# lbcb-sci/raven

Hardware: NVIDIA H100
Metric: overlaps/s (higher is better)
Workload: dtype u64

## Files before the change

raven_b200/csrc/map.cu:

```cuda
#include <algorithm>

#include "engine.cuh"

namespace rvn {

namespace {

constexpr int kThreads = 256;

struct IndexView {
  ValView val;
  const uint64_t* org;
  const uint32_t* bucket;
  uint64_t n;
  int shift;
  uint32_t occurrence;
  uint64_t limit;
};

__device__ __forceinline__ void Lookup(const IndexView& ix, uint64_t v,
                                       uint32_t* first, uint32_t* count) {
  if (v > ix.limit) {
    *first = 0;
    *count = 0;
// ... 39 lines not shown

__global__ void __launch_bounds__(kThreads)
ProbeKernel(IndexView ix, ValView q_val,
            const uint64_t* __restrict__ q_org, uint64_t q_begin, uint64_t n_q,
            bool avoid_equal, bool avoid_symmetric,
            uint32_t* __restrict__ cnt, uint32_t* __restrict__ first,
            uint8_t* __restrict__ filt) {
  const uint64_t i = static_cast<uint64_t>(blockIdx.x) * kThreads + threadIdx.x;
  if (i >= n_q) return;
  const uint64_t v = q_val[q_begin + i];
  const uint32_t lhs_id = static_cast<uint32_t>(q_org[q_begin + i] >> 32);
  uint32_t f, n;
  Lookup(ix, v, &f, &n);
  uint32_t kept = 0;
  uint8_t over = 0;
  if (n > ix.occurrence) {
    over = 1;
    n = 0;
  } else {
    for (uint32_t j = 0; j < n; ++j) {
      kept += KeepPosting(lhs_id, ix.org[f + j], avoid_equal, avoid_symmetric);
    }
  }
  cnt[i] = kept;
  first[i] = f;
  filt[i] = over;
}

__global__ void __launch_bounds__(kThreads)
ExpandKernel(IndexView ix, ValView q_val,
             const uint64_t* __restrict__ q_org, uint64_t q_begin, uint64_t n_q,
             bool avoid_equal, bool avoid_symmetric,
             const uint32_t* __restrict__ cnt,
             const uint32_t* __restrict__ first,
             const uint64_t* __restrict__ hit_off, uint64_t* __restrict__ h_grp,
             uint64_t* __restrict__ h_pos) {
  const uint64_t i = static_cast<uint64_t>(blockIdx.x) * kThreads + threadIdx.x;
  if (i >= n_q) return;
  uint32_t left = cnt[i];
  if (left == 0) return;
  const uint64_t v = q_val[q_begin + i];
  const uint64_t lo = q_org[q_begin + i];
  const uint32_t lhs_id = static_cast<uint32_t>(lo >> 32);
  const uint64_t lhs_pos = static_cast<uint32_t>(lo) >> 1;
  uint64_t dst = hit_off[i];
  for (uint64_t j = first[i]; left > 0 && j < ix.n && ix.val[j] == v; ++j) {
    const uint64_t o = ix.org[j];
    if (!KeepPosting(lhs_id, o, avoid_equal, avoid_symmetric)) continue;
    const uint64_t rhs_id = o >> 32;
    const uint64_t strand = (lo & 1) == (o & 1);
    const uint64_t rhs_pos = static_cast<uint32_t>(o) >> 1;
    const uint64_t diagonal =
        !strand ? rhs_pos + lhs_pos : rhs_pos - lhs_pos + (3ULL << 30);
    h_grp[dst] = (((rhs_id << 1) | strand) << 32) | diagonal;
    h_pos[dst] = (lhs_pos << 32) | rhs_pos;
    ++dst;
    --left;
  }
}

__global__ void __launch_bounds__(kThreads)
ProbeSuffixKernel(IndexView ix, ValView q_val,
                  const uint64_t* __restrict__ q_org, uint64_t q_begin, uint64_t n_q,
                  bool strict_above, uint32_t* __restrict__ cnt,
                  uint32_t* __restrict__ first, uint8_t* __restrict__ filt) {
  const uint64_t i = static_cast<uint64_t>(blockIdx.x) * kThreads + threadIdx.x;
  if (i >= n_q) return;
  const uint64_t v = q_val[q_begin + i];
  uint32_t f, n;
  Lookup(ix, v, &f, &n);
  uint8_t over = 0;
  uint32_t kept = 0, fk = f;
  if (n > ix.occurrence) {
    over = 1;
  } else if (n > 0) {
    if (strict_above) {
      const uint32_t lhs_id = static_cast<uint32_t>(q_org[q_begin + i] >> 32);
      uint32_t lo = f, hi = f + n;
      while (lo < hi) {
        const uint32_t mid = lo + (hi - lo) / 2;
        if (static_cast<uint32_t>(ix.org[mid] >> 32) <= lhs_id) lo = mid + 1; else hi = mid;
      }
      fk = lo;
    }
    kept = f + n - fk;
  }
  cnt[i] = kept;
  first[i] = fk;
  filt[i] = over;
}

__global__ void __launch_bounds__(kThreads)
ProbeSortedKernel(IndexView ix, ValView sorted_val,
                  const uint32_t* __restrict__ sorted_idx,
                  const uint64_t* __restrict__ q_org, uint64_t q_begin, uint64_t n_q,
                  bool strict_above, uint64_t* __restrict__ packed) {
  const uint64_t t = static_cast<uint64_t>(blockIdx.x) * kThreads + threadIdx.x;
  if (t >= n_q) return;
  const uint64_t v = sorted_val[t];
  const uint32_t i = sorted_idx[t];
  uint32_t f, n;
  Lookup(ix, v, &f, &n);
  uint8_t over = 0;
  uint32_t kept = 0, fk = f;
  if (n > ix.occurrence) {
    over = 1;
  } else if (n > 0) {
    if (strict_above) {
      const uint32_t lhs_id = static_cast<uint32_t>(q_org[q_begin + i] >> 32);
      uint32_t lo = f, hi = f + n;
      while (lo < hi) {
        const uint32_t mid = lo + (hi - lo) / 2;
        if (static_cast<uint32_t>(ix.org[mid] >> 32) <= lhs_id) lo = mid + 1; else hi = mid;
      }
      fk = lo;
    }
    kept = f + n - fk;
  }
  packed[i] = (static_cast<uint64_t>(fk) << 32) | (static_cast<uint64_t>(over) << 31) | kept;
}

__global__ void UnpackProbe(const uint64_t* __restrict__ packed, uint64_t n,
                            uint32_t* __restrict__ cnt, uint32_t* __restrict__ first,
                            uint8_t* __restrict__ filt) {
  const uint64_t i = static_cast<uint64_t>(blockIdx.x) * blockDim.x + threadIdx.x;
  if (i >= n) return;
  const uint64_t p = packed[i];
  cnt[i] = static_cast<uint32_t>(p) & 0x7FFFFFFFu;
  first[i] = static_cast<uint32_t>(p >> 32);
  filt[i] = static_cast<uint8_t>((p >> 31) & 1);
}


__global__ void __launch_bounds__(kThreads)
ExpandWarpKernel(IndexView ix, const uint64_t* __restrict__ q_org, uint64_t q_begin,
                 uint64_t n_q, const uint32_t* __restrict__ cnt,
                 const uint32_t* __restrict__ first, const uint64_t* __restrict__ hit_off,
                 uint64_t* __restrict__ h_grp, uint64_t* __restrict__ h_pos) {
  const uint32_t lane = threadIdx.x & 31;
  const uint64_t i = (static_cast<uint64_t>(blockIdx.x) * kThreads + threadIdx.x);
  const bool valid = i < n_q;
  const uint32_t my_cnt = valid ? cnt[i] : 0;
  const uint32_t my_first = valid ? first[i] : 0;
  const uint64_t my_org = valid ? q_org[q_begin + i] : 0;
  const uint64_t my_off = valid ? hit_off[i] : 0;
  const uint64_t base = __shfl_sync(0xFFFFFFFFu, my_off, 0);
  uint32_t rel = valid ? static_cast<uint32_t>(my_off - base) : 0;
  uint32_t run = valid ? rel + my_cnt : 0;
  for (int d = 1; d < 32; d <<= 1) {
    const uint32_t o = __shfl_up_sync(0xFFFFFFFFu, run, d);
    if (lane >= d && o > run) run = o;
  }
  if (!valid) rel = run;
  const uint32_t total = __shfl_sync(0xFFFFFFFFu, run, 31);
  for (uint32_t t0 = 0; t0 < total; t0 += 32) {
    const uint32_t t = t0 + lane;
    uint32_t q = 0;
#pragma unroll
    for (uint32_t step = 16; step > 0; step >>= 1) {
      const uint32_t r = __shfl_sync(0xFFFFFFFFu, rel, q + step);
      if (r <= t) q += step;
    }
    const uint32_t qrel = __shfl_sync(0xFFFFFFFFu, rel, q);
    const uint32_t qfirst = __shfl_sync(0xFFFFFFFFu, my_first, q);
    const uint64_t lo = __shfl_sync(0xFFFFFFFFu, my_org, q);
    if (t < total) {
      const uint64_t o = ix.org[qfirst + (t - qrel)];
      const uint64_t lhs_pos = static_cast<uint32_t>(lo) >> 1;
      const uint64_t rhs_id = o >> 32;
      const uint64_t strand = (lo & 1) == (o & 1);
      const uint64_t rhs_pos = static_cast<uint32_t>(o) >> 1;
      const uint64_t diagonal =
          !strand ? rhs_pos + lhs_pos : rhs_pos - lhs_pos + (3ULL << 30);
      h_grp[base + t] = (((rhs_id << 1) | strand) << 32) | diagonal;
      h_pos[base + t] = (lhs_pos << 32) | rhs_pos;
    }
  }
}

struct JoinView {
  ValView val;
  const uint64_t* org;
  uint64_t n;
  uint32_t occurrence;
  const uint64_t* thr_val;
  const uint32_t* thr_pos;
  uint32_t first, last;
};

__device__ __forceinline__ bool JoinIsQuery(const JoinView& jv, uint64_t v, uint64_t o) {
  const uint32_t r = static_cast<uint32_t>(o >> 32);
  if (r < jv.first || r >= jv.last) return false;
  const uint64_t t = jv.thr_val[r - jv.first];
  return v < t || (v == t && (static_cast<uint32_t>(o) >> 1) < jv.thr_pos[r - jv.first]);
}

template <typename Pred>
__device__ __forceinline__ uint64_t WarpFirst(uint64_t lo, uint64_t hi, uint32_t lane,
                                              Pred past) {
  while (lo < hi) {
    const uint64_t step = (hi - lo + 31) / 32;
    const uint64_t p = lo + (lane + 1) * step - 1;
    const uint32_t b = __ballot_sync(0xFFFFFFFFu, p >= hi || past(p));
    if (!b) return hi;
    const uint64_t f = __ffs(b) - 1;
    hi = min(hi, lo + (f + 1) * step - 1);
    lo += f * step;
  }
  return lo;
}

__global__ void __launch_bounds__(kThreads)
JoinSweepKernel(JoinView jv, const uint64_t* __restrict__ q_off,
                uint32_t* __restrict__ cursor, uint64_t* __restrict__ packed) {
  constexpr uint32_t kAll = 0xFFFFFFFFu;
  const uint32_t lane = threadIdx.x & 31;
  const uint64_t base = (static_cast<uint64_t>(blockIdx.x) * kThreads + threadIdx.x) & ~31ULL;
  if (base >= jv.n) return;
  const uint64_t i = base + lane;
  const bool valid = i < jv.n;
  const uint64_t v = valid ? jv.val[i] : 0;
  const uint64_t o = valid ? jv.org[i] : 0;
  const uint32_t r = static_cast<uint32_t>(o >> 32);
  const bool q = valid && JoinIsQuery(jv, v, o);
  if (!__any_sync(kAll, q)) return;

  uint64_t vn = __shfl_down_sync(kAll, v, 1);
  uint32_t rn = __shfl_down_sync(kAll, r, 1);
  uint64_t vp = __shfl_up_sync(kAll, v, 1);
  const bool has_next = i + 1 < jv.n;
  if (lane == 31 && has_next) {
    vn = jv.val[i + 1];
    rn = static_cast<uint32_t>(jv.org[i + 1] >> 32);
  }
  if (lane == 0 && i > 0) vp = jv.val[i - 1];
  const bool run_tail = !has_next || vn != v;
  const uint32_t tails = __ballot_sync(kAll, run_tail);
  const uint32_t seg_tails = __ballot_sync(kAll, run_tail || rn != r);
  const uint32_t heads = __ballot_sync(kAll, i == 0 || vp != v);
  const uint32_t at_or_above = kAll << lane, at_or_below = kAll >> (31 - lane);
  uint64_t run_end = (tails & at_or_above) ? base + __ffs(tails & at_or_above) : 0;
  uint64_t seg_end = (seg_tails & at_or_above) ? base + __ffs(seg_tails & at_or_above) : 0;
  bool over = false;
  const bool limited = jv.occurrence != kAll;

  if (__any_sync(kAll, q && run_end == 0)) {
    const uint64_t vl = __shfl_sync(kAll, v, 31);
    const uint32_t rl = __shfl_sync(kAll, r, 31);
    const uint64_t j = base + 32, k = j + lane;
    const bool dv = k >= jv.n || jv.val[k] != vl;
    const uint32_t bv = __ballot_sync(kAll, dv);
    const uint32_t bs =
        __ballot_sync(kAll, dv || static_cast<uint32_t>(jv.org[k] >> 32) != rl);
    uint64_t e_run = bv ? j + __ffs(bv) - 1 : 0;
    bool o_fw = false;
    if (!bv) {
      if (limited && 33 > jv.occurrence) {
        o_fw = true;
      } else {
        const uint64_t hi = limited ? min(jv.n, base + 32 + jv.occurrence) : jv.n;
        e_run = WarpFirst(j + 32, hi, lane, [&](uint64_t p) { return jv.val[p] != vl; });
        o_fw = e_run == hi && hi < jv.n && jv.val[hi] == vl;
      }
    }
    uint64_t e_seg = bs ? j + __ffs(bs) - 1 : 0;
    if (!bs && !o_fw) {
      e_seg = WarpFirst(j + 32, e_run, lane, [&](uint64_t p) {
        return static_cast<uint32_t>(jv.org[p] >> 32) != rl;
      });
    }
    if (run_end == 0) {
      run_end = e_run;
      over = o_fw;
    }
    if (seg_end == 0) seg_end = e_seg;
  }
  uint32_t run_start =
      (heads & at_or_below) ? static_cast<uint32_t>(base) + 31 - __clz(heads & at_or_below) : 0;
  if (limited && __any_sync(kAll, q && !over && !(heads & at_or_below))) {
    const uint64_t vf = __shfl_sync(kAll, v, 0);
    const uint64_t e0 = __shfl_sync(kAll, run_end, 0);
    const int64_t j = static_cast<int64_t>(base) - 32, k = j + lane;
    const uint32_t bv = __ballot_sync(kAll, k < 0 || jv.val[k] != vf);
    uint64_t s_run;
    if (bv) {
      s_run = static_cast<uint64_t>(j + 32 - __clz(bv));
    } else {
      const uint64_t lo = e0 > jv.occurrence + 1ULL ? e0 - jv.occurrence - 1 : 0;
      s_run = lo >= static_cast<uint64_t>(j)
                  ? static_cast<uint64_t>(j)
                  : WarpFirst(lo, static_cast<uint64_t>(j), lane,
                              [&](uint64_t p) { return jv.val[p] == vf; });
    }
    if (!(heads & at_or_below)) run_start = static_cast<uint32_t>(s_run);
  }
  if (!q || over || (limited && run_end - run_start > jv.occurrence)) return;
  const uint32_t kept = static_cast<uint32_t>(run_end - seg_end);
  if (!kept) return;
  const uint32_t rr = r - jv.first;
  const uint64_t slot = q_off[rr] + atomicAdd(cursor + rr, 1u);
  packed[slot] = (i << 32) | kept;
}

__global__ void UnpackJoin(const uint64_t* __restrict__ packed, uint64_t n,
                           uint32_t* __restrict__ cnt) {
  const uint64_t i = static_cast<uint64_t>(blockIdx.x) * blockDim.x + threadIdx.x;
  if (i < n) cnt[i] = static_cast<uint32_t>(packed[i]);
}

__global__ void __launch_bounds__(kThreads)
ExpandJoinKernel(const uint64_t* __restrict__ i_org, const uint64_t* __restrict__ packed,
                 uint64_t n_q, const uint64_t* __restrict__ hit_off,
                 uint64_t* __restrict__ h_grp, uint64_t* __restrict__ h_pos) {
  const uint32_t lane = threadIdx.x & 31;
  const uint64_t i = (static_cast<uint64_t>(blockIdx.x) * kThreads + threadIdx.x);
  const bool valid = i < n_q;
  const uint64_t pk = valid ? packed[i] : 0;
  const uint32_t my_cnt = static_cast<uint32_t>(pk);
  uint32_t my_first = 0;
  uint64_t my_org = 0;
  if (my_cnt) {
    const uint32_t post = static_cast<uint32_t>(pk >> 32);
    my_org = i_org[post];
    my_first = post + 1;
    while ((i_org[my_first] >> 32) == (my_org >> 32)) ++my_first;
  }
  const uint64_t my_off = valid ? hit_off[i] : 0;
  const uint64_t base = __shfl_sync(0xFFFFFFFFu, my_off, 0);
  uint32_t rel = valid ? static_cast<uint32_t>(my_off - base) : 0;
  uint32_t run = valid ? rel + my_cnt : 0;
  for (int d = 1; d < 32; d <<= 1) {
    const uint32_t o = __shfl_up_sync(0xFFFFFFFFu, run, d);
    if (lane >= d && o > run) run = o;
  }
  if (!valid) rel = run;
  const uint32_t total = __shfl_sync(0xFFFFFFFFu, run, 31);
  for (uint32_t t0 = 0; t0 < total; t0 += 32) {
    const uint32_t t = t0 + lane;
    uint32_t q = 0;
#pragma unroll
    for (uint32_t step = 16; step > 0; step >>= 1) {
      const uint32_t r = __shfl_sync(0xFFFFFFFFu, rel, q + step);
      if (r <= t) q += step;
    }
    const uint32_t qrel = __shfl_sync(0xFFFFFFFFu, rel, q);
    const uint32_t qfirst = __shfl_sync(0xFFFFFFFFu, my_first, q);
    const uint64_t lo = __shfl_sync(0xFFFFFFFFu, my_org, q);
    if (t < total) {
      const uint64_t o = i_org[qfirst + (t - qrel)];
      const uint64_t lhs_pos = static_cast<uint32_t>(lo) >> 1;
      const uint64_t rhs_id = o >> 32;
      const uint64_t strand = (lo & 1) == (o & 1);
      const uint64_t rhs_pos = static_cast<uint32_t>(o) >> 1;
      const uint64_t diagonal =
          !strand ? rhs_pos + lhs_pos : rhs_pos - lhs_pos + (3ULL << 30);
      h_grp[base + t] = (((rhs_id << 1) | strand) << 32) | diagonal;
      h_pos[base + t] = (lhs_pos << 32) | rhs_pos;
    }
  }
}

__global__ void GatherU64(const uint64_t* __restrict__ src,
                          const uint64_t* __restrict__ idx, uint64_t idx_base,
                          uint64_t n, uint64_t* __restrict__ dst) {
  const uint64_t i = static_cast<uint64_t>(blockIdx.x) * blockDim.x + threadIdx.x;
  if (i >= n) return;
  dst[i] = src[idx[i] - idx_base];
}

__global__ void FilteredFlagsToU32(const uint8_t* __restrict__ filt, uint64_t n,
                                   uint32_t* __restrict__ out) {
  const uint64_t i = static_cast<uint64_t>(blockIdx.x) * blockDim.x + threadIdx.x;
  if (i < n) out[i] = filt[i];
}
__global__ void ScatterFiltered(const uint8_t* __restrict__ filt,
                                const uint64_t* __restrict__ pos,
                                const uint64_t* __restrict__ q_org,
                                uint64_t q_begin, uint64_t n,
                                uint32_t* __restrict__ out) {
  const uint64_t i = static_cast<uint64_t>(blockIdx.x) * blockDim.x + threadIdx.x;
  if (i >= n || !filt[i]) return;
  out[pos[i]] = static_cast<uint32_t>(q_org[q_begin + i]) >> 1;
}


struct ChainParams {
  uint32_t k, bandwidth, chain, matches, gap;
};

template <int THREADS>
__device__ void BitonicSortPairs(uint64_t* A, uint64_t* B, uint32_t npad) {
  for (uint32_t size = 2; size <= npad; size <<= 1) {
    for (uint32_t stride = size >> 1; stride > 0; stride >>= 1) {
      for (uint32_t t = threadIdx.x; t < (npad >> 1); t += THREADS) {
        const uint32_t i = 2 * t - (t & (stride - 1));
        const uint32_t j = i + stride;
        const bool up = (i & size) == 0;
        const uint64_t ai = A[i], aj = A[j], bi = B[i], bj = B[j];
        const bool gt = ai > aj || (ai == aj && bi > bj);
        if (gt == up) {
          A[i] = aj;
          A[j] = ai;
          B[i] = bj;
          B[j] = bi;
        }
      }
      __syncthreads();
    }
  }
}

template <typename IdxT>
struct ChainWork {
  uint64_t* G;
  uint64_t* P;
  IdxT* LB;
  IdxT* PD;
  IdxT* IB;
  IdxT* IE;
  uint32_t* CNT;
};

template <typename IdxT, int THREADS>
__device__ uint32_t ChainRead(const ChainWork<IdxT>& wk, uint32_t n,
                              uint32_t npad, uint32_t lhs_id,
                              const ChainParams& cp, uint32_t* sm32,
                              rvn_overlap* __restrict__ ovl_raw,
                              unsigned long long* __restrict__ ovl_counter,
                              uint64_t ovl_cap, uint64_t* out_base,
                              uint64_t* __restrict__ ovl_key = nullptr, uint64_t key_hi = 0) {
  uint64_t* G = wk.G;
  uint64_t* P = wk.P;
  __shared__ unsigned long long sh_base;

  BitonicSortPairs<THREADS>(G, P, npad);

  for (uint32_t i = threadIdx.x; i <= n; i += THREADS) {
    const uint64_t gi = i < n ? G[i] : ~0ULL;
    uint32_t lo = 0, hi = i;
    while (lo < hi) {
      const uint32_t mid = lo + (hi - lo) / 2;
      if (gi - G[mid] <= cp.bandwidth) {
        hi = mid;
      } else {
        lo = mid + 1;
      }
    }
    wk.LB[i] = static_cast<IdxT>(lo);
  }
  __syncthreads();

  uint32_t carry_prevq = 0;
  uint32_t carry_nb = 0;
  for (uint32_t base = 1; base <= n; base += THREADS) {
    const uint32_t i = base + threadIdx.x;
    uint32_t e = 0, jp = 0;
    if (i <= n) {
      jp = wk.LB[i - 1];
      const uint64_t gi = i < n ? G[i] : ~0ULL;
      e = (gi - G[jp] > cp.bandwidth) && (i - jp >= 4);
    }
    const uint32_t incl = BlockInclusiveMax<uint32_t, THREADS>(e ? i : 0u, sm32);
    uint32_t prevq_incl_before;
    {
      __shared__ uint32_t sh_incl[THREADS];
      sh_incl[threadIdx.x] = incl;
      __syncthreads();
      prevq_incl_before = threadIdx.x ? sh_incl[threadIdx.x - 1] : 0u;
      __syncthreads();
    }
    const uint32_t prevq = max(carry_prevq, prevq_incl_before);
    const uint32_t start = e && (prevq == 0 || prevq <= jp);
    uint32_t tot;
    const uint32_t ex = BlockExclusiveSum<uint32_t, THREADS>(start, sm32, &tot);
    if (e) {
      const uint32_t band = carry_nb + ex + start - 1;
      if (start) {
        wk.IB[band] = static_cast<IdxT>(jp);
        if (prevq != 0) wk.IE[band - 1] = static_cast<IdxT>(prevq);
      }
    }
    carry_nb += tot;
    {
      __shared__ uint32_t sh_last;
      if (threadIdx.x == THREADS - 1) sh_last = max(carry_prevq, incl);
      __syncthreads();
      carry_prevq = sh_last;
      __syncthreads();
    }
  }
  const uint32_t nb = carry_nb;
  if (threadIdx.x == 0 && nb) wk.IE[nb - 1] = static_cast<IdxT>(carry_prevq);
  __syncthreads();
  if (nb == 0) return 0;

  for (uint32_t i = threadIdx.x; i < npad; i += THREADS) {
    if (i >= n) {
      G[i] = ~0ULL;
      continue;
    }
    uint32_t lo = 0, hi = nb;
    while (lo < hi) {
      const uint32_t mid = lo + (hi - lo) / 2;
      if (wk.IB[mid] <= i) {
        lo = mid + 1;
      } else {
        hi = mid;
      }
    }
    uint64_t tag;
    if (lo == 0) {
      tag = 0;
    } else if (i < wk.IE[lo - 1]) {
      tag = 2ULL * (lo - 1) + 1;
    } else {
      tag = 2ULL * lo;
    }
    G[i] = (tag << 32) | (G[i] >> 32);
  }
  __syncthreads();
  BitonicSortPairs<THREADS>(G, P, npad);

  IdxT* MINI = wk.LB;
  for (uint32_t b = threadIdx.x; b < nb; b += THREADS) {
    const uint32_t jb = wk.IB[b], ie = wk.IE[b];
    const uint32_t len = ie - jb;
    uint32_t emitted = 0;
    uint32_t longest = 0;
    if (len >= cp.chain) {
      const uint64_t* Pb = P + jb;
      IdxT* minimal = MINI + jb + b;
      IdxT* pred = wk.PD + jb;
      const bool strand = G[jb] & 1;
      minimal[0] = 0;
      for (uint32_t t = 0; t < len; ++t) {
        const uint32_t cl = static_cast<uint32_t>(Pb[t] >> 32);
        const uint32_t cr = static_cast<uint32_t>(Pb[t]);
        uint32_t lo = 1, hi = longest;
        while (lo <= hi) {
          const uint32_t mid = lo + (hi - lo) / 2;
          const uint64_t tail = Pb[minimal[mid]];
          const uint32_t tl = static_cast<uint32_t>(tail >> 32);
          const uint32_t tr = static_cast<uint32_t>(tail);
          if (tl < cl && (strand ? tr < cr : tr > cr)) {
            lo = mid + 1;
          } else {
            hi = mid - 1;
          }
        }
        pred[t] = minimal[lo - 1];
        minimal[lo] = static_cast<IdxT>(t);
        longest = max(longest, lo);
      }
      if (longest >= cp.chain) {
        uint32_t j = minimal[longest];
        for (uint32_t i = 0; i < longest; ++i) {
          const uint32_t pj = pred[j];
          minimal[longest - 1 - i] = static_cast<IdxT>(j);
          j = pj;
        }
      } else {
        longest = 0;
      }
    }
    if (longest) {
      const uint64_t* Pb = P + jb;
      const IdxT* idx = MINI + jb + b;
      const bool strand = G[jb] & 1;
      for (uint32_t kk = 1, l = 0; kk <= longest; ++kk) {
        const uint32_t prev = static_cast<uint32_t>(Pb[idx[kk - 1]] >> 32);
        const uint32_t cur =
            kk < longest ? static_cast<uint32_t>(Pb[idx[kk]] >> 32) : 0xFFFFFFFFu;
        if (cur - prev > cp.gap) {
          if (kk - l >= cp.chain) {
            uint32_t lm = 0, lb_ = 0, le = 0, rm = 0, rb_ = 0, re = 0;
            for (uint32_t m = l; m < kk; ++m) {
              const uint64_t pp = Pb[idx[m]];
              const uint32_t lp = static_cast<uint32_t>(pp >> 32);
              if (lp > le) {
                lm += le - lb_;
                lb_ = lp;
              }
              le = lp + cp.k;
              uint32_t rp = static_cast<uint32_t>(pp);
              rp = strand ? rp : (1U << 31) - (rp + cp.k - 1);
              if (rp > re) {
                rm += re - rb_;
                rb_ = rp;
              }
              re = rp + cp.k;
            }
            lm += le - lb_;
            rm += re - rb_;
            if (min(lm, rm) >= cp.matches) ++emitted;
          }
          l = kk;
        }
      }
    }
    wk.CNT[b] = emitted;
    wk.IE[b] = static_cast<IdxT>(longest);
  }
  __syncthreads();

  uint32_t carry = 0;
  __shared__ uint32_t sh_total;
  {
    uint32_t local = 0;
    for (uint32_t b = threadIdx.x; b < nb; b += THREADS) local += wk.CNT[b];
    uint32_t tot;
    BlockExclusiveSum<uint32_t, THREADS>(local, sm32, &tot);
    if (threadIdx.x == 0) {
      sh_total = tot;
      sh_base = tot ? atomicAdd(ovl_counter, static_cast<unsigned long long>(tot))
                    : 0ULL;
    }
    __syncthreads();
  }
  const uint32_t total = sh_total;
  const uint64_t base = sh_base;
  *out_base = base;
  if (total == 0 || base + total > ovl_cap) return total;

  for (uint32_t b0 = 0; b0 < nb; b0 += THREADS) {
    const uint32_t b = b0 + threadIdx.x;
    const uint32_t mine = b < nb ? wk.CNT[b] : 0;
    uint32_t tot;
    const uint32_t ex = BlockExclusiveSum<uint32_t, THREADS>(mine, sm32, &tot);
    if (mine) {
      rvn_overlap* dst = ovl_raw + base + carry + ex;
      uint64_t* kdst = ovl_key ? ovl_key + base + carry + ex : nullptr;
      uint32_t seq = carry + ex;
      const uint32_t jb = wk.IB[b];
      const uint32_t longest = wk.IE[b];
      const uint64_t* Pb = P + jb;
      const IdxT* idx = MINI + jb + b;
      const bool strand = G[jb] & 1;
      const uint32_t rhs_id = static_cast<uint32_t>(G[jb] & 0xFFFFFFFFu) >> 1;
      for (uint32_t kk = 1, l = 0; kk <= longest; ++kk) {
        const uint32_t prev = static_cast<uint32_t>(Pb[idx[kk - 1]] >> 32);
        const uint32_t cur =
            kk < longest ? static_cast<uint32_t>(Pb[idx[kk]] >> 32) : 0xFFFFFFFFu;
        if (cur - prev > cp.gap) {
          if (kk - l >= cp.chain) {
            uint32_t lm = 0, lb_ = 0, le = 0, rm = 0, rb_ = 0, re = 0;
            for (uint32_t m = l; m < kk; ++m) {
              const uint64_t pp = Pb[idx[m]];
              const uint32_t lp = static_cast<uint32_t>(pp >> 32);
              if (lp > le) {
                lm += le - lb_;
                lb_ = lp;
              }
              le = lp + cp.k;
              uint32_t rp = static_cast<uint32_t>(pp);
              rp = strand ? rp : (1U << 31) - (rp + cp.k - 1);
              if (rp > re) {
                rm += re - rb_;
                rb_ = rp;
              }
              re = rp + cp.k;
            }
// ... 551 lines not shown
  const uint64_t i = static_cast<uint64_t>(blockIdx.x) * blockDim.x + threadIdx.x;
  if (i < n) cnt[i] = static_cast<uint32_t>(ovl_loc[i] & 0xFFFFFF);
}

__global__ void ReorderOverlaps(const rvn_overlap* __restrict__ raw,
                                const uint64_t* __restrict__ ovl_loc,
                                const uint64_t* __restrict__ ovl_off,
                                uint32_t n_reads, rvn_overlap* __restrict__ out) {
  const uint32_t r = blockIdx.x * (blockDim.x / 32) + (threadIdx.x >> 5);
  if (r >= n_reads) return;
  const uint64_t loc = ovl_loc[r];
  const uint32_t cnt = static_cast<uint32_t>(loc & 0xFFFFFF);
  const uint64_t src = loc >> 24, dst = ovl_off[r];
  const uint4* s = reinterpret_cast<const uint4*>(raw + src);
  uint4* d = reinterpret_cast<uint4*>(out + dst);
  for (uint32_t i = threadIdx.x & 31; i < cnt * 2; i += 32) d[i] = s[i];
}

void JoinSweep(Ctx& c, uint32_t first) {
  const uint32_t nr = c.i_last - first;
  const uint64_t t0 = first - c.qt_first, base = c.h_q_off[t0];
  c.h_j_off.resize(nr + 1ULL);
  for (uint32_t i = 0; i <= nr; ++i) c.h_j_off[i] = c.h_q_off[t0 + i] - base;
  const uint64_t n_q = c.h_j_off[nr];
  uint64_t* off = c.j_off.reserve(nr + 1ULL);
  RVN_CUDA(cudaMemcpyAsync(off, c.h_j_off.data(), (nr + 1ULL) * sizeof(uint64_t),
                           cudaMemcpyHostToDevice, c.stream));
  uint32_t* cursor = c.j_cursor.reserve(nr + 1ULL);
  uint64_t* packed = c.j_packed.reserve(n_q + 1);
  RVN_CUDA(cudaMemsetAsync(cursor, 0, (nr + 1ULL) * sizeof(uint32_t), c.stream));
  RVN_CUDA(cudaMemsetAsync(packed, 0, (n_q + 1) * sizeof(uint64_t), c.stream));
  if (c.i_n > 0 && n_q > 0) {
    JoinView jv{ValView{c.i_val.get(), c.i_is32 ? 1 : 0}, c.i_org.get(), c.i_n, c.occurrence,
                c.qt_val.get() + t0, c.qt_pos.get() + t0, first, c.i_last};
    JoinSweepKernel<<<CeilDiv(c.i_n, kThreads), kThreads, 0, c.stream>>>(jv, off, cursor,
                                                                          packed);
    RVN_LAUNCH_CHECK();
    ++c.launches;
  }
  RVN_CUDA(cudaStreamSynchronize(c.stream));
  c.j_gen = c.i_gen;
  c.j_occurrence = c.occurrence;
  c.j_first = first;
}

}

uint64_t ChainGroupedHits(Ctx& c, const uint64_t* hg, const uint64_t* hp,
                          const uint64_t* read_hit_off,
                          const std::vector<uint64_t>& h_rho, const uint32_t* lhs_ids,
                          uint32_t nr, uint64_t n_hits, uint64_t n_q) {
  TimerBegin(c, "chain");
  ChainParams cp{c.prm.k, c.prm.bandwidth, c.prm.chain, c.prm.matches, c.prm.gap};
  const uint64_t ovl_cap = n_hits / std::max(1u, std::min(c.prm.chain, 4u)) + 16;
  rvn_overlap* raw = c.m_ovl_raw.reserve(ovl_cap);
  uint64_t* loc = c.m_ovl_loc.reserve(nr + 1ULL);
  uint64_t* counter = c.m_counter.reserve((1u << 16) + 8);
  RVN_CUDA(cudaMemsetAsync(counter, 0, sizeof(uint64_t), c.stream));
  RVN_CUDA(cudaMemsetAsync(loc, 0, (nr + 1ULL) * sizeof(uint64_t), c.stream));

  static const uint32_t kBounds[] = {256, 512, 1024, 2048, 4096, 8192, 65536};
  constexpr int kClasses = sizeof(kBounds) / sizeof(kBounds[0]);
  std::vector<uint32_t> cls[kClasses];
  std::vector<uint32_t> big;
  const bool fast_ok = c.prm.chain >= 1;
  for (uint32_t i = 0; i < nr; ++i) {
    const uint64_t n = h_rho[i + 1] - h_rho[i];
    if (n < 4) continue;
    if (n > kChainSmemCap || !fast_ok) {
      big.push_back(i);
      continue;
    }
    int k = 0;
    while (kBounds[k] < n + 1) ++k;
    cls[k].push_back(i);
  }
  uint64_t n_fast_ovl = 0;
  {
    size_t total = 0;
    for (auto& v : cls) total += v.size();
    uint32_t* d_list = c.m_first.reserve(std::max<size_t>(total, n_q) + 1);
    uint32_t* d_fb = c.m_fallback.reserve(nr + 4ULL);
    RVN_CUDA(cudaMemsetAsync(d_fb, 0, 2 * sizeof(uint32_t), c.stream));
    std::vector<uint32_t> flat;
    flat.reserve(total);
    for (int k = kClasses - 1; k >= 0; --k) {
      flat.insert(flat.end(), cls[k].begin(), cls[k].end());
    }
    if (total) {
      RVN_CUDA(cudaMemcpyAsync(d_list, flat.data(), total * sizeof(uint32_t),
                               cudaMemcpyHostToDevice, c.stream));
      RVN_CUDA(cudaStreamSynchronize(c.stream));

      const uint64_t max_groups = n_hits / 4 + 1;
      GroupDesc* desc = reinterpret_cast<GroupDesc*>(
          c.m_desc.reserve(max_groups * (sizeof(GroupDesc) / 4)));
      uint32_t* dcnt = c.m_desc_cnt.reserve(max_groups);
      uint32_t* didx = c.m_desc_idx.reserve(max_groups);
      uint32_t* dcnt2 = c.m_desc_cnt2.reserve(max_groups);
      uint32_t* didx2 = c.m_desc_idx2.reserve(max_groups);
      uint32_t* g_diag = c.m_gdiag.reserve(n_hits + 1);
      uint64_t* g_pos = c.m_gpos.reserve(n_hits + 1);
      uint64_t* group_loc = c.m_group_loc.reserve(nr + 1ULL);
      RVN_CUDA(cudaMemsetAsync(counter, 0, 4 * sizeof(uint64_t), c.stream));
      auto* ctr = reinterpret_cast<unsigned long long*>(counter);

      size_t off = 0;
      for (int k = kClasses - 1; k >= 0; --k) {
        const unsigned cnt = static_cast<unsigned>(cls[k].size());
        if (cnt == 0) continue;
        const size_t smem = MakeSplitLayout(kBounds[k] - 1).bytes;
        const uint32_t* lst = d_list + off;
        off += cnt;
        if (kBounds[k] > 2048) {
          auto kern = SplitKernel<256, 2>;
          RVN_CUDA(cudaFuncSetAttribute(
              kern, cudaFuncAttributeMaxDynamicSharedMemorySize,
              static_cast<int>(MakeSplitLayout(kChainSmemCap).bytes)));
          kern<<<cnt, 256, smem, c.stream>>>(hg, hp, read_hit_off, lhs_ids, lst,
                                             ctr + 1, desc, dcnt, didx, g_diag, g_pos,
                                             group_loc, d_fb + 2, d_fb);
        } else {
          auto kern = SplitKernel<128, 8>;
          kern<<<cnt, 128, smem, c.stream>>>(hg, hp, read_hit_off, lhs_ids, lst,
                                             ctr + 1, desc, dcnt, didx, g_diag, g_pos,
                                             group_loc, d_fb + 2, d_fb);
        }
        RVN_LAUNCH_CHECK();
        ++c.launches;
      }
      uint64_t* hpin = c.pin64.reserve(8);
      RVN_CUDA(cudaMemcpyAsync(hpin, counter, 4 * sizeof(uint64_t),
                               cudaMemcpyDeviceToHost, c.stream));
      std::vector<uint32_t> fb(2);
      RVN_CUDA(cudaMemcpyAsync(fb.data(), d_fb, 2 * sizeof(uint32_t),
                               cudaMemcpyDeviceToHost, c.stream));
      RVN_CUDA(cudaStreamSynchronize(c.stream));
      const uint64_t n_groups = hpin[1];
      const uint32_t nfb = fb[0];
      if (nfb) {
        fb.resize(nfb);
        RVN_CUDA(cudaMemcpyAsync(fb.data(), d_fb + 2, nfb * sizeof(uint32_t),
                                 cudaMemcpyDeviceToHost, c.stream));
        RVN_CUDA(cudaStreamSynchronize(c.stream));
        std::sort(fb.begin(), fb.end());
        big.insert(big.end(), fb.begin(), fb.end());
      }
      if (n_groups >= 0xFFFFFFFFULL) throw LimitError("2^32 or more seed pairs");
      if (hpin[2] >= 0xFFFFFFFFULL) throw LimitError("2^32 or more chained seed hits in one flush");

      if (n_groups) {
        const int w_desc = RadixSortPairs(c, dcnt, dcnt2, dcnt, didx, didx2, didx, n_groups, 0, 13,
                                          true);
        const uint32_t* sorted_cnt = w_desc == 0 ? dcnt2 : dcnt;
        const uint32_t* sorted_idx = w_desc == 0 ? didx2 : didx;
        rvn_overlap* tmp_ovl = c.m_ovl_tmp.reserve(ovl_cap);
        uint64_t* key = c.m_okey.reserve(ovl_cap);
        uint64_t* key2 = c.m_okey2.reserve(ovl_cap);
        uint32_t* oidx = c.m_oidx.reserve(ovl_cap);
        uint32_t* oidx2 = c.m_oidx2.reserve(ovl_cap);
        static const uint32_t kGB[] = {8191, 4095, 2047, 1023, 511, 255, 127, 63,
                                       kThreadPairMax, 32, 24, 16, 8};
        constexpr uint32_t kNB = sizeof(kGB) / sizeof(kGB[0]);
        constexpr uint32_t kFirstThreadClass = 8;
        uint32_t* d_bounds = c.m_bounds.reserve(kNB);
        uint64_t* d_starts = c.m_starts.reserve(kNB + 1);
        RVN_CUDA(cudaMemcpyAsync(d_bounds, kGB, sizeof(kGB), cudaMemcpyHostToDevice,
                                 c.stream));
        SizeClassStarts<<<1, 32, 0, c.stream>>>(sorted_cnt, n_groups, d_bounds, kNB, d_starts);
        uint64_t h_starts[kNB + 1];
        RVN_CUDA(cudaMemcpyAsync(h_starts, d_starts, kNB * sizeof(uint64_t),
                                 cudaMemcpyDeviceToHost, c.stream));
        RVN_CUDA(cudaStreamSynchronize(c.stream));
        h_starts[kNB] = n_groups;
        h_starts[0] = 0;
        RVN_CUDA(cudaFuncSetAttribute(GroupChainKernel,
                                      cudaFuncAttributeMaxDynamicSharedMemorySize,
                                      200 * 1024));
        RVN_CUDA(cudaFuncSetAttribute(PairChainKernel,
                                      cudaFuncAttributeMaxDynamicSharedMemorySize,
                                      static_cast<int>(PairChainSmem(8192))));
        for (uint32_t b = 0; b < kNB; ++b) {
          const uint64_t lo = h_starts[b], hi = h_starts[b + 1];
          if (hi <= lo) continue;
          if (b < kFirstThreadClass) {
            const uint32_t npad = kGB[b] + 1;
            PairChainKernel<<<static_cast<unsigned>(hi - lo), kPairThreads, PairChainSmem(npad),
                              c.stream>>>(desc, sorted_idx, lo, npad, g_diag, g_pos, cp, tmp_ovl,
                                          key, ctr + 3, ovl_cap);
          } else {
            uint32_t threads = 128;
            while (threads > 8 && 12ULL * kGB[b] * threads > 196 * 1024) threads >>= 1;
            const size_t smem = 12ULL * kGB[b] * threads;
            GroupChainKernel<<<CeilDiv(hi - lo, threads), threads, smem, c.stream>>>(
                desc, sorted_idx, lo, hi, kGB[b], g_diag, g_pos, cp, tmp_ovl, key, ctr + 3,
                ovl_cap);
          }
          RVN_LAUNCH_CHECK();
          ++c.launches;
        }
        n_fast_ovl = ReadU64(c, counter + 3);
        if (n_fast_ovl > ovl_cap) throw LimitError("overlap slab overflow");
        if (n_fast_ovl >= 0xFFFFFFFFULL) throw LimitError("2^32 or more overlaps");
        if (n_fast_ovl) {
          IotaU32<<<CeilDiv(n_fast_ovl, kThreads), kThreads, 0, c.stream>>>(
              oidx, n_fast_ovl);
          int key_bits = 17;
          while (key_bits < 64 && (1ULL << (key_bits - 16)) < n_groups) ++key_bits;
          const int w_ovl = RadixSortPairs(c, key, key2, key, oidx, oidx2, oidx, n_fast_ovl, 0,
                                           key_bits);
          const uint64_t* sorted_key = w_ovl == 0 ? key2 : key;
          const uint32_t* sorted_oidx = w_ovl == 0 ? oidx2 : oidx;
          GatherOverlapsByIndex<<<CeilDiv(n_fast_ovl * 2, kThreads), kThreads, 0,
                                  c.stream>>>(tmp_ovl, sorted_oidx, n_fast_ovl, raw);
          LocateReadOverlaps<<<CeilDiv(total, kThreads), kThreads, 0, c.stream>>>(
              sorted_key, n_fast_ovl, d_list, static_cast<uint32_t>(total),
              group_loc, 0, loc);
          RVN_LAUNCH_CHECK();
          c.launches += 3;
        }
      }
      RVN_CUDA(cudaMemcpyAsync(counter, &n_fast_ovl, sizeof(uint64_t),
                               cudaMemcpyHostToDevice, c.stream));
      RVN_CUDA(cudaStreamSynchronize(c.stream));
    }
  }
  if (!big.empty()) {
    std::vector<uint64_t> off64(big.size() + 1, 0), off32(big.size() + 1, 0);
    for (size_t i = 0; i < big.size(); ++i) {
      const uint64_t n = h_rho[big[i] + 1] - h_rho[big[i]];
      if (n >= 0x7FFFFFFFULL) throw LimitError("a query has 2^31 or more hits");
      uint64_t npad = 8;
      while (npad < n + 1) npad <<= 1;
      const uint64_t nbmax = n / 4 + 1;
      off64[i + 1] = off64[i] + 2 * npad;
      off32[i + 1] = off32[i] + (n + nbmax + 2) + (n + 1) + 3 * nbmax + 4;
    }
    uint64_t* slab64 = c.m_scratch64.reserve(off64.back() + 2 * (big.size() + 1) + 8);
    uint32_t* slab32 = c.m_scratch32.reserve(off32.back() + big.size() + 8);
    uint64_t* d_off64 = slab64 + off64.back();
    uint64_t* d_off32 = d_off64 + big.size() + 1;
    uint32_t* d_big = slab32 + off32.back();
    RVN_CUDA(cudaMemcpyAsync(d_off64, off64.data(), (big.size() + 1) * 8,
                             cudaMemcpyHostToDevice, c.stream));
    RVN_CUDA(cudaMemcpyAsync(d_off32, off32.data(), (big.size() + 1) * 8,
                             cudaMemcpyHostToDevice, c.stream));
    RVN_CUDA(cudaMemcpyAsync(d_big, big.data(), big.size() * 4,
                             cudaMemcpyHostToDevice, c.stream));
    ChainKernelGlobal<<<static_cast<unsigned>(big.size()), kThreads, 0,
                        c.stream>>>(
        hg, hp, read_hit_off, lhs_ids, d_big, d_off64, d_off32, slab64, slab32, cp,
        raw, reinterpret_cast<unsigned long long*>(counter), ovl_cap, loc);
    RVN_LAUNCH_CHECK();
    ++c.launches;
    RVN_CUDA(cudaStreamSynchronize(c.stream));
  }

  uint32_t* ocnt = c.m_cnt.reserve(nr + 1ULL);
  uint64_t* ooff = c.m_ovl_off.reserve(nr + 2ULL);
  uint64_t n_ovl = 0;
  if (nr > 0) {
    OverlapCounts<<<CeilDiv(nr, kThreads), kThreads, 0, c.stream>>>(loc, nr, ocnt);
    RVN_LAUNCH_CHECK();
    ++c.launches;
    ExclusiveScanU32(c, ocnt, ooff, nr);
    n_ovl = ReadU64(c, ooff + nr);
  } else {
    RVN_CUDA(cudaMemsetAsync(ooff, 0, sizeof(uint64_t), c.stream));
  }
  if (n_ovl > ovl_cap) throw LimitError("overlap slab overflow");
  rvn_overlap* ordered = c.m_ovl.reserve(n_ovl + 1);
  if (n_ovl > 0) {
    ReorderOverlaps<<<CeilDiv(nr, kThreads / 32), kThreads, 0, c.stream>>>(
        raw, loc, ooff, nr, ordered);
    RVN_LAUNCH_CHECK();
    ++c.launches;
  }
  TimerEnd(c);
  return n_ovl;
}

void MapRange(Ctx& c, uint32_t first, uint32_t last, bool avoid_equal,
              bool avoid_symmetric, bool minhash, bool want_filtered,
              bool fetch) {
  if (!c.i_valid) throw StateError("Map before Minimize");
  c.r_valid = false;
  const uint32_t nr = last - first;

  const bool join = c.self_join && minhash && avoid_equal && avoid_symmetric && !want_filtered &&
                    c.i_from_sketch && c.i_sorted_ids && c.ids_identity && first >= c.i_first &&
                    last <= c.i_last;
  uint64_t n_q = 0, n_hits = 0;
  uint64_t *hg = nullptr, *hp = nullptr;
  uint64_t* read_hit_off = c.m_read_hit_off.reserve(nr + 2ULL);
  std::vector<uint64_t> h_rho(nr + 1ULL);
  if (join) {
    const bool sweep = c.j_gen != c.i_gen || c.j_occurrence != c.occurrence || first < c.j_first;
    if (sweep && !(c.qt_valid && c.qt_first <= first && c.i_last <= c.qt_last)) {
      EnsureThresholds(c, first, c.i_last);
    }
    TimerBegin(c, "probe");
    if (sweep) JoinSweep(c, first);
    const uint64_t b0 = first - c.j_first;
    const uint64_t q_begin = c.h_j_off[b0];
    n_q = c.h_j_off[b0 + nr] - q_begin;
    const uint64_t* packed = c.j_packed.get() + q_begin;
    uint64_t* hit_off = c.m_hit_off.reserve(n_q + 2);
    if (n_q > 0) {
      uint32_t* cnt = c.m_cnt.reserve(n_q + 1);
      UnpackJoin<<<CeilDiv(n_q, kThreads), kThreads, 0, c.stream>>>(packed, n_q, cnt);
      RVN_LAUNCH_CHECK();
      ++c.launches;
      ExclusiveScanU32(c, cnt, hit_off, n_q);
      n_hits = ReadU64(c, hit_off + n_q);
    } else {
      RVN_CUDA(cudaMemsetAsync(hit_off, 0, sizeof(uint64_t), c.stream));
    }
    TimerEnd(c);
    TimerBegin(c, "expand");
    hg = c.h_grp.reserve(n_hits + 1);
    hp = c.h_pos.reserve(n_hits + 1);
    if (n_hits > 0) {
      ExpandJoinKernel<<<CeilDiv(n_q, kThreads), kThreads, 0, c.stream>>>(
          c.i_org.get(), packed, n_q, hit_off, hg, hp);
      RVN_LAUNCH_CHECK();
      ++c.launches;
    }
    GatherU64<<<CeilDiv(nr + 1ULL, kThreads), kThreads, 0, c.stream>>>(
        hit_off, c.j_off.get() + b0, q_begin, nr + 1ULL, read_hit_off);
    RVN_LAUNCH_CHECK();
    ++c.launches;
    RVN_CUDA(cudaMemcpyAsync(h_rho.data(), read_hit_off, (nr + 1ULL) * sizeof(uint64_t),
                             cudaMemcpyDeviceToHost, c.stream));
    RVN_CUDA(cudaStreamSynchronize(c.stream));
    TimerEnd(c);
    c.r_filt_off.reserve(nr + 2ULL);
    for (uint32_t i = 0; i <= nr; ++i) c.r_filt_off.get()[i] = 0;
  } else {
  const uint64_t *qo, *d_read_off;
  ValView qv;
  const std::vector<uint64_t>* h_read_off;
  uint64_t off_base_read;
  if (minhash) {
    if (!(c.q_valid && c.q_first <= first && last <= c.q_last)) {
      EnsureMicromizers(c, first, last);
    }
    qv = ValView{c.q_val.get(), c.q_is32 ? 1 : 0};
    qo = c.q_org.get();
    d_read_off = c.q_off.get();
    h_read_off = &c.h_q_off;
    off_base_read = first - c.q_first;
  } else {
    if (!(c.s_valid && c.s_first <= first && last <= c.s_last)) {
      EnsureSketch(c, first, last);
    }
    qv = ValView{c.s_val.get(), c.s_is32 ? 1 : 0};
    qo = c.s_org.get();
    d_read_off = c.s_off.get();
    h_read_off = &c.h_s_off;
    off_base_read = first - c.s_first;
  }
  const uint64_t q_begin = (*h_read_off)[off_base_read];
  n_q = (*h_read_off)[off_base_read + nr] - q_begin;

  IndexView ix{ValView{c.i_val.get(), c.i_is32 ? 1 : 0}, c.i_org.get(), c.i_bucket.get(), c.i_n,
               c.i_shift, c.occurrence, c.i_limit};

  TimerBegin(c, "probe");
  uint32_t* cnt = c.m_cnt.reserve(n_q + 1);
  uint32_t* frst = c.m_first.reserve(n_q + 1);
  uint8_t* filt = c.m_filt.reserve(n_q + 1);
  uint64_t* hit_off = c.m_hit_off.reserve(n_q + 2);
  const bool suffix = (avoid_equal && avoid_symmetric && c.i_sorted_ids) ||
                      (!avoid_equal && !avoid_symmetric);
  if (n_q > 0) {
    if (suffix && n_q >= (1u << 16) && n_q < 0xFFFFFFFFULL) {
      uint64_t* k1 = c.m_sq_key.reserve(n_q + 2);
      uint64_t* k2 = c.m_sq_key2.reserve(n_q);
      uint32_t* v1 = c.m_sq_idx.reserve(n_q);
      uint32_t* v2 = c.m_sq_idx2.reserve(n_q);
      IotaU32<<<CeilDiv(n_q, kThreads), kThreads, 0, c.stream>>>(v1, n_q);
      const int hi_bit = static_cast<int>(2 * c.prm.k);
      int w_q;
      ValView sorted_qv;
      if (qv.is32) {
        const uint32_t* src = static_cast<const uint32_t*>(qv.p) + q_begin;
        uint32_t* a32 = reinterpret_cast<uint32_t*>(k1);
        uint32_t* b32 = a32 + n_q + (n_q & 1);
        w_q = RadixSortPairs(c, src, a32, b32, v1, v2, v1, n_q, 0, hi_bit);
        sorted_qv = ValView{w_q < 0 ? src : (w_q == 0 ? a32 : b32), 1};
      } else {
        const uint64_t* src = static_cast<const uint64_t*>(qv.p) + q_begin;
        w_q = RadixSortPairs(c, src, k1, k2, v1, v2, v1, n_q, 0, hi_bit);
        sorted_qv = ValView{w_q < 0 ? src : (w_q == 0 ? k1 : k2), 0};
      }
      const uint32_t* sorted_qi = w_q == 0 ? v2 : v1;
      uint64_t* packed = (qv.is32 || w_q == 0) ? k2 : k1;
      ProbeSortedKernel<<<CeilDiv(n_q, kThreads), kThreads, 0, c.stream>>>(
          ix, sorted_qv, sorted_qi, qo, q_begin, n_q, avoid_equal, packed);
      UnpackProbe<<<CeilDiv(n_q, kThreads), kThreads, 0, c.stream>>>(packed, n_q, cnt, frst, filt);
      c.launches += (2 * c.prm.k + 7) / 8 + 5;
    } else if (suffix) {
      ProbeSuffixKernel<<<CeilDiv(n_q, kThreads), kThreads, 0, c.stream>>>(
          ix, qv, qo, q_begin, n_q, avoid_equal, cnt, frst, filt);
    } else {
      ProbeKernel<<<CeilDiv(n_q, kThreads), kThreads, 0, c.stream>>>(
          ix, qv, qo, q_begin, n_q, avoid_equal, avoid_symmetric, cnt, frst, filt);
    }
    RVN_LAUNCH_CHECK();
    ++c.launches;
    ExclusiveScanU32(c, cnt, hit_off, n_q);
    n_hits = ReadU64(c, hit_off + n_q);
  } else {
    RVN_CUDA(cudaMemsetAsync(hit_off, 0, sizeof(uint64_t), c.stream));
  }
  TimerEnd(c);
  TimerBegin(c, "expand");
  hg = c.h_grp.reserve(n_hits + 1);
  hp = c.h_pos.reserve(n_hits + 1);
  if (n_hits > 0) {
    if (suffix) {
      ExpandWarpKernel<<<CeilDiv(n_q, kThreads), kThreads, 0, c.stream>>>(
          ix, qo, q_begin, n_q, cnt, frst, hit_off, hg, hp);
    } else {
      ExpandKernel<<<CeilDiv(n_q, kThreads), kThreads, 0, c.stream>>>(
          ix, qv, qo, q_begin, n_q, avoid_equal, avoid_symmetric, cnt, frst,
          hit_off, hg, hp);
    }
    RVN_LAUNCH_CHECK();
    ++c.launches;
  }
  GatherU64<<<CeilDiv(nr + 1ULL, kThreads), kThreads, 0, c.stream>>>(
      hit_off, d_read_off + off_base_read, q_begin, nr + 1ULL, read_hit_off);
  RVN_LAUNCH_CHECK();
  ++c.launches;
  RVN_CUDA(cudaMemcpyAsync(h_rho.data(), read_hit_off,
                           (nr + 1ULL) * sizeof(uint64_t),
                           cudaMemcpyDeviceToHost, c.stream));
  RVN_CUDA(cudaStreamSynchronize(c.stream));
  TimerEnd(c);

  c.r_filt_off.reserve(nr + 2ULL);
  for (uint32_t i = 0; i <= nr; ++i) c.r_filt_off.get()[i] = 0;
  uint64_t n_filtered = 0;
  if (want_filtered && n_q > 0) {
    uint32_t* f32 = c.m_first.get();
    FilteredFlagsToU32<<<CeilDiv(n_q, kThreads), kThreads, 0, c.stream>>>(
        filt, n_q, f32);
    uint64_t* fpos = c.m_filt_off.reserve(n_q + 2);
    ExclusiveScanU32(c, f32, fpos, n_q);
    n_filtered = ReadU64(c, fpos + n_q);
    uint32_t* fout = c.m_filtered.reserve(n_filtered + 1);
    ScatterFiltered<<<CeilDiv(n_q, kThreads), kThreads, 0, c.stream>>>(
        filt, fpos, qo, q_begin, n_q, fout);
    RVN_LAUNCH_CHECK();
    c.launches += 2;
    uint64_t* froff = c.m_ovl_off.reserve(nr + 2ULL);
    GatherU64<<<CeilDiv(nr + 1ULL, kThreads), kThreads, 0, c.stream>>>(
        fpos, d_read_off + off_base_read, q_begin, nr + 1ULL, froff);
    RVN_LAUNCH_CHECK();
    ++c.launches;
    uint32_t* hf = c.r_filtered.reserve(n_filtered + 1);
    RVN_CUDA(cudaMemcpyAsync(hf, fout, n_filtered * sizeof(uint32_t),
                             cudaMemcpyDeviceToHost, c.stream));
    RVN_CUDA(cudaMemcpyAsync(c.r_filt_off.get(), froff,
                             (nr + 1ULL) * sizeof(uint64_t),
                             cudaMemcpyDeviceToHost, c.stream));
    RVN_CUDA(cudaStreamSynchronize(c.stream));
  }

  }

  if (c.keep_hits) {
    uint64_t* g = c.r_hit_grp.reserve(n_hits + 1);
    uint64_t* p = c.r_hit_pos.reserve(n_hits + 1);
    uint64_t* o = c.r_hit_off.reserve(nr + 2ULL);
    RVN_CUDA(cudaMemcpyAsync(g, hg, n_hits * sizeof(uint64_t),
                             cudaMemcpyDeviceToHost, c.stream));
    RVN_CUDA(cudaMemcpyAsync(p, hp, n_hits * sizeof(uint64_t),
                             cudaMemcpyDeviceToHost, c.stream));
    for (uint32_t i = 0; i <= nr; ++i) o[i] = h_rho[i];
    RVN_CUDA(cudaStreamSynchronize(c.stream));
    c.r_n_hits = n_hits;
  }

  const uint64_t n_ovl =
      ChainGroupedHits(c, hg, hp, read_hit_off, h_rho, c.d_ids.get() + first, nr, n_hits, n_q);
  const rvn_overlap* ordered = c.m_ovl.get();
  const uint64_t* ooff = c.m_ovl_off.get();

  if (fetch) {
    rvn_overlap* ho = c.r_ovl.reserve(n_ovl + 1);
    uint64_t* hoff = c.r_ovl_off.reserve(nr + 2ULL);
    RVN_CUDA(cudaMemcpyAsync(ho, ordered, n_ovl * sizeof(rvn_overlap),
                             cudaMemcpyDeviceToHost, c.stream));
    RVN_CUDA(cudaMemcpyAsync(hoff, ooff, (nr + 1ULL) * sizeof(uint64_t),
                             cudaMemcpyDeviceToHost, c.stream));
    RVN_CUDA(cudaStreamSynchronize(c.stream));
  }
  c.r_n_ovl = n_ovl;
  c.m_hits = n_hits;
  c.m_first_read = first;
  c.m_last_read = last;
  c.r_valid = fetch;

  uint64_t qbases = 0;
  for (uint32_t r = first; r < last; ++r) qbases += c.h_len[r];
  c.stats.query_bases += qbases;
  c.stats.query_records += n_q;
  c.stats.hits += n_hits;
  c.stats.overlaps += n_ovl;
}

}
```

Before: 53.82 million.

## Expand self-join hits per read with block-level scan instead of per-slot scan

The join expansion now works per read instead of per query slot. A warp-per-read kernel sums each read's hit counts and a scan over reads gives the read hit offsets directly. ExpandJoinKernel then runs one block per read, uses a block exclusive sum and a shared-memory binary search to map output indices to slots, and writes each read's hits contiguously. This drops the large per-slot scan over n_q, the gather kernel and one device-to-host readback. In exchange, reads with few slots leave most of a 256-thread block idle, and each block synchronises for every chunk of slots.

```diff
diff --git a/raven_b200/csrc/map.cu b/raven_b200/csrc/map.cu
--- a/raven_b200/csrc/map.cu
+++ b/raven_b200/csrc/map.cu
@@ -365,61 +365,67 @@
   packed[slot] = (i << 32) | kept;
 }
 
-__global__ void UnpackJoin(const uint64_t* __restrict__ packed, uint64_t n,
-                           uint32_t* __restrict__ cnt) {
-  const uint64_t i = static_cast<uint64_t>(blockIdx.x) * blockDim.x + threadIdx.x;
-  if (i < n) cnt[i] = static_cast<uint32_t>(packed[i]);
+__global__ void JoinReadHits(const uint64_t* __restrict__ slots,
+                             const uint64_t* __restrict__ slot_off, uint32_t nr,
+                             uint32_t* __restrict__ cnt) {
+  const uint32_t r = (blockIdx.x * blockDim.x + threadIdx.x) >> 5, lane = threadIdx.x & 31;
+  if (r >= nr) return;
+  uint32_t s = 0;
+  for (uint64_t i = slot_off[r] + lane; i < slot_off[r + 1]; i += 32) {
+    s += static_cast<uint32_t>(slots[i]);
+  }
+  for (int d = 16; d > 0; d >>= 1) s += __shfl_down_sync(0xFFFFFFFFu, s, d);
+  if (lane == 0) cnt[r] = s;
 }
 
 __global__ void __launch_bounds__(kThreads)
-ExpandJoinKernel(const uint64_t* __restrict__ i_org, const uint64_t* __restrict__ packed,
-                 uint64_t n_q, const uint64_t* __restrict__ hit_off,
+ExpandJoinKernel(const uint64_t* __restrict__ i_org, const uint64_t* __restrict__ slots,
+                 const uint64_t* __restrict__ slot_off, const uint64_t* __restrict__ read_hit_off,
                  uint64_t* __restrict__ h_grp, uint64_t* __restrict__ h_pos) {
-  const uint32_t lane = threadIdx.x & 31;
-  const uint64_t i = (static_cast<uint64_t>(blockIdx.x) * kThreads + threadIdx.x);
-  const bool valid = i < n_q;
-  const uint64_t pk = valid ? packed[i] : 0;
-  const uint32_t my_cnt = static_cast<uint32_t>(pk);
-  uint32_t my_first = 0;
-  uint64_t my_org = 0;
-  if (my_cnt) {
-    const uint32_t post = static_cast<uint32_t>(pk >> 32);
-    my_org = i_org[post];
-    my_first = post + 1;
-    while ((i_org[my_first] >> 32) == (my_org >> 32)) ++my_first;
-  }
-  const uint64_t my_off = valid ? hit_off[i] : 0;
-  const uint64_t base = __shfl_sync(0xFFFFFFFFu, my_off, 0);
-  uint32_t rel = valid ? static_cast<uint32_t>(my_off - base) : 0;
-  uint32_t run = valid ? rel + my_cnt : 0;
-  for (int d = 1; d < 32; d <<= 1) {
-    const uint32_t o = __shfl_up_sync(0xFFFFFFFFu, run, d);
-    if (lane >= d && o > run) run = o;
-  }
-  if (!valid) rel = run;
-  const uint32_t total = __shfl_sync(0xFFFFFFFFu, run, 31);
-  for (uint32_t t0 = 0; t0 < total; t0 += 32) {
-    const uint32_t t = t0 + lane;
-    uint32_t q = 0;
+  __shared__ uint32_t sm32[34];
+  __shared__ uint32_t sh_rel[kThreads], sh_first[kThreads], sh_lo[kThreads];
+  const uint32_t r = blockIdx.x;
+  const uint64_t hb = read_hit_off[r];
+  if (read_hit_off[r + 1] == hb) return;
+  const uint64_t* sl = slots + slot_off[r];
+  const uint32_t n_slots = static_cast<uint32_t>(slot_off[r + 1] - slot_off[r]);
+  uint64_t* hg = h_grp + hb;
+  uint64_t* hp = h_pos + hb;
+  uint32_t done = 0;
+  for (uint32_t c0 = 0; c0 < n_slots; c0 += kThreads) {
+    const uint32_t s = c0 + threadIdx.x;
+    const uint64_t pk = s < n_slots ? sl[s] : 0;
+    const uint32_t cnt = static_cast<uint32_t>(pk);
+    uint32_t tot;
+    const uint32_t ex = BlockExclusiveSum<uint32_t, kThreads>(cnt, sm32, &tot);
+    if (cnt) {
+      const uint32_t post = static_cast<uint32_t>(pk >> 32);
+      const uint64_t org = i_org[post];
+      uint32_t first = post + 1;
+      while ((i_org[first] >> 32) == (org >> 32)) ++first;
+      sh_first[threadIdx.x] = first;
+      sh_lo[threadIdx.x] = static_cast<uint32_t>(org);
+    }
+    sh_rel[threadIdx.x] = ex;
+    __syncthreads();
+    for (uint32_t t = threadIdx.x; t < tot; t += kThreads) {
+      uint32_t q = 0;
 #pragma unroll
-    for (uint32_t step = 16; step > 0; step >>= 1) {
-      const uint32_t r = __shfl_sync(0xFFFFFFFFu, rel, q + step);
-      if (r <= t) q += step;
-    }
-    const uint32_t qrel = __shfl_sync(0xFFFFFFFFu, rel, q);
-    const uint32_t qfirst = __shfl_sync(0xFFFFFFFFu, my_first, q);
-    const uint64_t lo = __shfl_sync(0xFFFFFFFFu, my_org, q);
-    if (t < total) {
-      const uint64_t o = i_org[qfirst + (t - qrel)];
-      const uint64_t lhs_pos = static_cast<uint32_t>(lo) >> 1;
+      for (uint32_t step = kThreads / 2; step > 0; step >>= 1) {
+        if (sh_rel[q + step] <= t) q += step;
+      }
+      const uint64_t o = i_org[sh_first[q] + (t - sh_rel[q])];
+      const uint64_t lhs_pos = sh_lo[q] >> 1;
       const uint64_t rhs_id = o >> 32;
-      const uint64_t strand = (lo & 1) == (o & 1);
+      const uint64_t strand = (sh_lo[q] & 1) == (o & 1);
       const uint64_t rhs_pos = static_cast<uint32_t>(o) >> 1;
       const uint64_t diagonal =
           !strand ? rhs_pos + lhs_pos : rhs_pos - lhs_pos + (3ULL << 30);
-      h_grp[base + t] = (((rhs_id << 1) | strand) << 32) | diagonal;
-      h_pos[base + t] = (lhs_pos << 32) | rhs_pos;
-    }
+      hg[done + t] = (((rhs_id << 1) | strand) << 32) | diagonal;
+      hp[done + t] = (lhs_pos << 32) | rhs_pos;
+    }
+    done += tot;
+    __syncthreads();
   }
 }
 
@@ -1577,37 +1583,32 @@
     TimerBegin(c, "probe");
     if (sweep) JoinSweep(c, first);
     const uint64_t b0 = first - c.j_first;
-    const uint64_t q_begin = c.h_j_off[b0];
-    n_q = c.h_j_off[b0 + nr] - q_begin;
-    const uint64_t* packed = c.j_packed.get() + q_begin;
-    uint64_t* hit_off = c.m_hit_off.reserve(n_q + 2);
-    if (n_q > 0) {
-      uint32_t* cnt = c.m_cnt.reserve(n_q + 1);
-      UnpackJoin<<<CeilDiv(n_q, kThreads), kThreads, 0, c.stream>>>(packed, n_q, cnt);
+    n_q = c.h_j_off[b0 + nr] - c.h_j_off[b0];
+    const uint64_t* slot_off = c.j_off.get() + b0;
+    if (nr > 0) {
+      uint32_t* cnt = c.m_cnt.reserve(nr + 1ULL);
+      JoinReadHits<<<CeilDiv(nr, kThreads / 32), kThreads, 0, c.stream>>>(c.j_packed.get(),
+                                                                          slot_off, nr, cnt);
       RVN_LAUNCH_CHECK();
       ++c.launches;
-      ExclusiveScanU32(c, cnt, hit_off, n_q);
-      n_hits = ReadU64(c, hit_off + n_q);
+      ExclusiveScanU32(c, cnt, read_hit_off, nr);
     } else {
-      RVN_CUDA(cudaMemsetAsync(hit_off, 0, sizeof(uint64_t), c.stream));
-    }
+      RVN_CUDA(cudaMemsetAsync(read_hit_off, 0, sizeof(uint64_t), c.stream));
+    }
+    RVN_CUDA(cudaMemcpyAsync(h_rho.data(), read_hit_off, (nr + 1ULL) * sizeof(uint64_t),
+                             cudaMemcpyDeviceToHost, c.stream));
+    RVN_CUDA(cudaStreamSynchronize(c.stream));
+    n_hits = h_rho[nr];
     TimerEnd(c);
     TimerBegin(c, "expand");
     hg = c.h_grp.reserve(n_hits + 1);
     hp = c.h_pos.reserve(n_hits + 1);
     if (n_hits > 0) {
-      ExpandJoinKernel<<<CeilDiv(n_q, kThreads), kThreads, 0, c.stream>>>(
-          c.i_org.get(), packed, n_q, hit_off, hg, hp);
+      ExpandJoinKernel<<<nr, kThreads, 0, c.stream>>>(c.i_org.get(), c.j_packed.get(), slot_off,
+                                                      read_hit_off, hg, hp);
       RVN_LAUNCH_CHECK();
       ++c.launches;
     }
-    GatherU64<<<CeilDiv(nr + 1ULL, kThreads), kThreads, 0, c.stream>>>(
-        hit_off, c.j_off.get() + b0, q_begin, nr + 1ULL, read_hit_off);
-    RVN_LAUNCH_CHECK();
-    ++c.launches;
-    RVN_CUDA(cudaMemcpyAsync(h_rho.data(), read_hit_off, (nr + 1ULL) * sizeof(uint64_t),
-                             cudaMemcpyDeviceToHost, c.stream));
-    RVN_CUDA(cudaStreamSynchronize(c.stream));
     TimerEnd(c);
     c.r_filt_off.reserve(nr + 2ULL);
     for (uint32_t i = 0; i <= nr; ++i) c.r_filt_off.get()[i] = 0;
```

New measurement: 56.54 million (median of 6 runs). 1.05x the previous value.
